# stcodeer/Frequency-wised_All-in-One_Image_Restoration_Model

Measured on AMD Instinct MI355X. Metric: training images/sec @128x128, higher is better.
Workload: dtype bf16; 1 GPU; BASELINE configs[1]: Uformer encoder+decoder (all_3_bands, L=3, freq MSA), denoise sigma=25, 128x128, phase-2 train step (fwd+bwd+Adam, DropPath on); per_gpu_batch=16, global_batch=16, parallelism=dp1, hip_graph=True

## Files before the change

frequency-wised_all-in-one_image_restoration_model_amd/csrc/fw_elem.hip:

```cpp
#include "fw_common.h"
#include <stdlib.h>

namespace {

constexpr int TPB = 256;
FW_DEV long gtid() { return (long)blockIdx.x * TPB + threadIdx.x; }
FW_DEV long gstride() { return (long)gridDim.x * TPB; }
static inline int grid_for(long n, int cap = 8192) { long g = (n + TPB - 1) / TPB; return (int)(g < 1 ? 1 : (g > cap ? cap : g)); }

template <typename T> FW_DEV void ldvec(const T* p, float* f) {
    unpack16<T>(*reinterpret_cast<const uint4*>(p), f);
}
template <typename T> FW_DEV void stvec(T* p, const float* f) { *reinterpret_cast<uint4*>(p) = pack16<T>(f); }
template <typename T> FW_DEV void ldvec4(const T* p, float* f);
template <> FW_SPEC void ldvec4<float>(const float* p, float* f) { unpack16<float>(*reinterpret_cast<const uint4*>(p), f); }
template <> FW_SPEC void ldvec4<bf16raw>(const bf16raw* p, float* f) {
    const uint2 v = *reinterpret_cast<const uint2*>(p);
    f[0] = __uint_as_float(v.x << 16); f[1] = __uint_as_float(v.x & 0xffff0000u);
    f[2] = __uint_as_float(v.y << 16); f[3] = __uint_as_float(v.y & 0xffff0000u);
}
template <typename T> FW_DEV void stvec4(T* p, const float* f);
template <> FW_SPEC void stvec4<float>(float* p, const float* f) { *reinterpret_cast<uint4*>(p) = pack16<float>(f); }
template <> FW_SPEC void stvec4<bf16raw>(bf16raw* p, const float* f) {
    *reinterpret_cast<uint2*>(p) = make_uint2(pack_bf2(f[0], f[1]), pack_bf2(f[2], f[3]));
// ... 654 lines not shown
            if (k < 9) atomicAdd(dw + (long)c * 9 + (8 - k), sum);
            else atomicAdd(dbias + c, sum);
        }
    }
}

template <typename T>
__global__ void im2col4_kernel(const float* __restrict__ x, long ldx, T* __restrict__ col, int B, int H, int W, int C) {
    const int Ho = H / 2, Wo = W / 2, c4n = C >> 2;
    const long total = (long)B * Ho * Wo * 16 * c4n;
    for (long i = gtid(); i < total; i += gstride()) {
        const int c = (int)(i % c4n) * 4; long t = i / c4n;
        const int tap = (int)(t % 16); t /= 16;
        const int ox = (int)(t % Wo); const int oy = (int)((t / Wo) % Ho); const long b = t / ((long)Wo * Ho);
        const int iy = 2 * oy - 1 + (tap >> 2), ix = 2 * ox - 1 + (tap & 3);
        f32x4 v = f32x4{0.f, 0.f, 0.f, 0.f};
        if (iy >= 0 && iy < H && ix >= 0 && ix < W) v = *reinterpret_cast<const f32x4*>(x + ((b * H + iy) * W + ix) * ldx + c);
        T* d = col + (t * 16 + tap) * (long)C + c;
        if (sizeof(T) == 4) *reinterpret_cast<f32x4*>(d) = v;
        else *reinterpret_cast<uint2*>(d) = make_uint2(pack_bf2(v[0], v[1]), pack_bf2(v[2], v[3]));
    }
}
template <typename T>
__global__ void col2im4_kernel(const T* __restrict__ dcol, float* __restrict__ dx, long lddx, const float* __restrict__ dres, long ldr,
                               int B, int H, int W, int C) {
    const int Ho = H / 2, Wo = W / 2, c4n = C >> 2;
    const long total = (long)B * H * W * c4n;
    for (long i = gtid(); i < total; i += gstride()) {
        const int c = (int)(i % c4n) * 4; const long tok = i / c4n;
        const int x = (int)(tok % W); const int y = (int)((tok / W) % H); const long b = tok / ((long)W * H);
        f32x4 acc = f32x4{0.f, 0.f, 0.f, 0.f};
        if (dres) acc = *reinterpret_cast<const f32x4*>(dres + tok * ldr + c);
        for (int ky = (y + 1) & 1; ky < 4; ky += 2) {
            const int oy = (y + 1 - ky) / 2;
            if (y + 1 - ky < 0 || oy >= Ho) continue;
            for (int kx = (x + 1) & 1; kx < 4; kx += 2) {
                const int ox = (x + 1 - kx) / 2;
                if (x + 1 - kx < 0 || ox >= Wo) continue;
                const T* s = dcol + (((b * Ho + oy) * Wo + ox) * 16 + ky * 4 + kx) * (long)C + c;
                for (int e = 0; e < 4; ++e) acc[e] += TT<T>::ld(s + e);
            }
        }
        *reinterpret_cast<f32x4*>(dx + tok * lddx + c) = acc;
    }
}

template <typename T>
__global__ void pixel_shuffle_kernel(const T* __restrict__ g, const float* __restrict__ bias, float* __restrict__ out, long ldo,
                                     int B, int H, int W, int Cout) {
    const int c4n = Cout >> 2;
    const long total = (long)B * H * W * 4 * c4n;
    for (long i = gtid(); i < total; i += gstride()) {
        const int c = (int)(i % c4n) * 4; long t = i / c4n;
        const int q = (int)(t % 4); t /= 4;
        const int x = (int)(t % W); const int y = (int)((t / W) % H); const long b = t / ((long)W * H);
        const T* s = g + t * 4L * Cout + q * Cout + c;
        float* d = out + ((b * 2 * H + 2 * y + (q >> 1)) * 2 * W + 2 * x + (q & 1)) * ldo + c;
        f32x4 v;
        for (int e = 0; e < 4; ++e) v[e] = TT<T>::ld(s + e) + bias[c + e];
        *reinterpret_cast<f32x4*>(d) = v;
    }
}
template <typename T>
__global__ void pixel_unshuffle_kernel(const float* __restrict__ dout, long ldo, T* __restrict__ dg, int B, int H, int W, int Cout) {
    const int c4n = Cout >> 2;
    const long total = (long)B * H * W * 4 * c4n;
// ... 50 lines not shown
    int tx, ty; long n;
    __device__ EcTiles(int B, int H, int W) : tx((W + EC_TX - 1) / EC_TX), ty((H + EC_TY - 1) / EC_TY) { n = (long)B * tx * ty; }
    __device__ void at(long t, long& b, int& y0, int& x0) const { x0 = (int)(t % tx) * EC_TX; y0 = (int)((t / tx) % ty) * EC_TY; b = t / ((long)tx * ty); }
};
FW_DEV void ec_patch_load(float (&r)[EC_PREG], const float* __restrict__ src, const EcTiles& T, long t, int H, int W) {
    long b; int y0, x0;
    T.at(t, b, y0, x0);
#pragma unroll
    for (int k = 0; k < EC_PREG; ++k) {
        int i = threadIdx.x + k * 256; i = i < EC_PN ? i : EC_PN - 1;
        const int ci = i / EC_PLANE, rem = i % EC_PLANE;
        const int y = y0 + rem / EC_PW - 1, x = x0 + rem % EC_PW - 1;
        const bool ok = y >= 0 && y < H && x >= 0 && x < W;
        const int yc = y < 0 ? 0 : (y >= H ? H - 1 : y), xc = x < 0 ? 0 : (x >= W ? W - 1 : x);
        const float v = src[((b * 3 + ci) * H + yc) * W + xc];
        r[k] = ok ? v : 0.f;
    }
}
FW_DEV void ec_patch_store(const float (&r)[EC_PREG], float* patch) {
#pragma unroll
    for (int k = 0; k < EC_PREG; ++k) { const int i = threadIdx.x + k * 256; if (i < EC_PN) patch[i] = r[k]; }
}

template <int MODE>
__global__ __launch_bounds__(256) void edge_conv3_rows_kernel(const float* __restrict__ src, const float* __restrict__ w, const float* __restrict__ bias,
                                                              float* __restrict__ out, long ldo, int B, int H, int W, int C, float slope) {
    __shared__ float patch[2][EC_PN];
    const int c4n = C >> 2, PL = 256 / c4n;
    const int q = threadIdx.x % c4n, pl = threadIdx.x / c4n;
    f32x4 wr[27], bq = f32x4{0.f, 0.f, 0.f, 0.f};
#pragma unroll
    for (int t = 0; t < 27; ++t)
#pragma unroll
        for (int e = 0; e < 4; ++e)
            wr[t][e] = MODE == 0 ? w[(4 * q + e) * 27 + t] : w[((long)(t / 9) * C + 4 * q + e) * 9 + 8 - t % 9];
    if (MODE == 0) bq = *reinterpret_cast<const f32x4*>(bias + 4 * q);
    const EcTiles T(B, H, W);
    float pr[EC_PREG];
    long t = blockIdx.x;
    if (t < T.n) { ec_patch_load(pr, src, T, t, H, W); ec_patch_store(pr, patch[0]); }
    __syncthreads();
    for (int cur = 0; t < T.n; t += gridDim.x, cur ^= 1) {
        const bool more = t + gridDim.x < T.n;
        if (more) ec_patch_load(pr, src, T, t + gridDim.x, H, W);
        long b; int y0, x0;
        T.at(t, b, y0, x0);
        const float* pc = patch[cur];
        if (pl < PL)
            for (int p = pl; p < EC_PIX; p += PL) {
                const int ty = p / EC_TX, tx = p % EC_TX, y = y0 + ty, x = x0 + tx;
                const float* pp = pc + ty * EC_PW + tx;
                f32x4 acc = bq;
#pragma unroll
                for (int ky = 0; ky < 3; ++ky)
#pragma unroll
                    for (int kx = 0; kx < 3; ++kx)
#pragma unroll
                        for (int ci = 0; ci < 3; ++ci) {
                            const int py = MODE == 0 ? ky : 2 - ky, px = MODE == 0 ? kx : 2 - kx;
                            acc += wr[ci * 9 + py * 3 + px] * pp[ci * EC_PLANE + py * EC_PW + px];
                        }
                if (MODE == 0)
#pragma unroll
                    for (int e = 0; e < 4; ++e) acc[e] = lrelu_f(acc[e], slope);
                if (y < H && x < W) *reinterpret_cast<f32x4*>(out + ((b * H + y) * W + x) * ldo + 4 * q) = acc;
            }
        if (more) ec_patch_store(pr, patch[cur ^ 1]);
        __syncthreads();
    }
}

template <int V, int MODE>
__global__ __launch_bounds__(256, 2) void edge_conv3_wgrad_kernel(const float* __restrict__ src, const float* __restrict__ a, long lda, const float* __restrict__ o,
                                                                  long ldo, float* __restrict__ dw, float* __restrict__ db, int B, int H, int W, int C, float slope) {
    constexpr int U = 4;
    __shared__ float patch[2][EC_PN];
    __shared__ float red[28 * 256];
    const int cvn = C / V, PL = 256 / cvn;
    const int q = threadIdx.x % cvn, pl = threadIdx.x / cvn;
    float g[27][V], gb[V];
#pragma unroll
    for (int e = 0; e < V; ++e) {
        gb[e] = 0.f;
#pragma unroll
        for (int t = 0; t < 27; ++t) g[t][e] = 0.f;
    }
    const EcTiles T(B, H, W);
    float pr[EC_PREG];
// ... 429 lines not shown
            ? dwconv_tile_launch<bf16raw, 1>((const bf16raw*)dh2, ldg, w, (const float*)nullptr, (const bf16raw*)h1, (bf16raw*)dh1, (bf16raw*)nullptr, ldo, B, H, W, C, ST)
            : dwconv_tile_launch<float, 1>((const float*)dh2, ldg, w, (const float*)nullptr, (const float*)h1, (float*)dh1, (float*)nullptr, ldo, B, H, W, C, ST);
        if (rc) return rc;
    }
    if (dtype == FW_DT_BF16) {
        if (!tiled) hipLaunchKernelGGL((dwconv_strip_kernel<bf16raw, 1>), dim3((grid_for(n) + 7) / 8 * 8), dim3(TPB), 0, ST, (const bf16raw*)dh2, ldg, w, (const float*)nullptr,
                           (const bf16raw*)h1, (bf16raw*)dh1, (bf16raw*)nullptr, ldo, B, H, W, C);
        if (g1) hipLaunchKernelGGL((dwconv_wgrad_kernel<bf16raw, false>), gridw, dim3(256), 0, ST, (const bf16raw*)dh2, ldg, (const bf16raw*)g1, ld1, dw, dbias, B, H, W, C, NSTRIP);
        else hipLaunchKernelGGL((dwconv_wgrad_kernel<bf16raw, true>), gridw, dim3(256), 0, ST, (const bf16raw*)dh2, ldg, (const bf16raw*)h1, ld1, dw, dbias, B, H, W, C, NSTRIP);
    } else {
        if (!tiled) hipLaunchKernelGGL((dwconv_strip_kernel<float, 1>), dim3((grid_for(n) + 7) / 8 * 8), dim3(TPB), 0, ST, (const float*)dh2, ldg, w, (const float*)nullptr,
                           (const float*)h1, (float*)dh1, (float*)nullptr, ldo, B, H, W, C);
        if (g1) hipLaunchKernelGGL((dwconv_wgrad_kernel<float, false>), gridw, dim3(256), 0, ST, (const float*)dh2, ldg, (const float*)g1, ld1, dw, dbias, B, H, W, C, NSTRIP);
        else hipLaunchKernelGGL((dwconv_wgrad_kernel<float, true>), gridw, dim3(256), 0, ST, (const float*)dh2, ldg, (const float*)h1, ld1, dw, dbias, B, H, W, C, NSTRIP);
    }
    FW_LAUNCH_RET();
}
extern "C" int fw_im2col4(int dtype, const float* x, long ldx, void* col, int B, int H, int W, int C, void* stream) {
    FW_CHECK_ARG(x && col && C % 4 == 0 && ldx % 4 == 0 && H % 2 == 0 && W % 2 == 0);
    const long n = (long)B * (H / 2) * (W / 2) * 16 * (C / 4);
    if (dtype == FW_DT_BF16) LAUNCH((im2col4_kernel<bf16raw>), n, x, ldx, (bf16raw*)col, B, H, W, C);
    LAUNCH((im2col4_kernel<float>), n, x, ldx, (float*)col, B, H, W, C);
}
extern "C" int fw_col2im4(int dtype, const void* dcol, float* dx, long lddx, const float* dres, long ldr, int B, int H, int W, int C,
                          void* stream) {
    FW_CHECK_ARG(dcol && dx && C % 4 == 0 && lddx % 4 == 0 && H % 2 == 0 && W % 2 == 0 && (!dres || ldr % 4 == 0));
    const long n = (long)B * H * W * (C / 4);
    if (dtype == FW_DT_BF16) LAUNCH((col2im4_kernel<bf16raw>), n, (const bf16raw*)dcol, dx, lddx, dres, ldr, B, H, W, C);
    LAUNCH((col2im4_kernel<float>), n, (const float*)dcol, dx, lddx, dres, ldr, B, H, W, C);
}
extern "C" int fw_pixel_shuffle(int dtype, const void* g, const float* bias, float* out, long ldo, int B, int H, int W, int Cout,
                                void* stream) {
    FW_CHECK_ARG(g && bias && out && Cout % 4 == 0 && ldo % 4 == 0);
    const long n = (long)B * H * W * Cout;
    if (dtype == FW_DT_BF16) LAUNCH((pixel_shuffle_kernel<bf16raw>), n, (const bf16raw*)g, bias, out, ldo, B, H, W, Cout);
    LAUNCH((pixel_shuffle_kernel<float>), n, (const float*)g, bias, out, ldo, B, H, W, Cout);
}
extern "C" int fw_pixel_unshuffle(int dtype, const float* dout, long ldo, void* dg, int B, int H, int W, int Cout, void* stream) {
    FW_CHECK_ARG(dout && dg && Cout % 4 == 0 && ldo % 4 == 0);
    const long n = (long)B * H * W * Cout;
    if (dtype == FW_DT_BF16) LAUNCH((pixel_unshuffle_kernel<bf16raw>), n, dout, ldo, (bf16raw*)dg, B, H, W, Cout);
    LAUNCH((pixel_unshuffle_kernel<float>), n, dout, ldo, (float*)dg, B, H, W, Cout);
}
extern "C" int fw_colsum(int x_dtype, const void* x, long ldx, float* out, long rows, int cols, void* stream) {
    FW_CHECK_ARG(x && out && rows > 0 && cols > 0);
    int rpb = (int)((rows + 1023) / 1024);
    if (rpb < 32) rpb = 32;
    int grid = (int)((rows + rpb - 1) / rpb);
    if (x_dtype != 1 && cols % 4 == 0 && cols <= 512 && ldx % 4 == 0 && ((uintptr_t)x & 15) == 0 && ((uintptr_t)out & 3) == 0) {
        rpb = (int)((rows + 255) / 256);
        if (rpb < 32) rpb = 32;
        grid = (int)((rows + rpb - 1) / rpb);
        hipLaunchKernelGGL(colsum4_kernel, dim3(grid), dim3(TPB), 0, ST, (const float*)x, ldx, out, rows, cols, rpb);
        FW_LAUNCH_RET();
    }
    if (x_dtype == 1) hipLaunchKernelGGL((colsum_t_kernel<bf16raw>), dim3(grid), dim3(TPB), 0, ST, (const bf16raw*)x, ldx, out, rows, cols, rpb);
    else hipLaunchKernelGGL(colsum_kernel, dim3(grid), dim3(TPB), 0, ST, (const float*)x, ldx, out, rows, cols, rpb);
    FW_LAUNCH_RET();
}
#ifndef FW_EC_WGRAD_CAP
#define FW_EC_WGRAD_CAP 512
#endif
static inline int ec_grid(int B, int H, int W, int cap) {
    const long n = (long)B * ((H + EC_TY - 1) / EC_TY) * ((W + EC_TX - 1) / EC_TX);
    return (int)(n < cap ? n : cap);
}
static inline bool ec_al16(const void* p) { return ((uintptr_t)p & 15) == 0; }
constexpr int OP_PROD_BYTES = ((EC_PLANE + 15) / 16) * 16 * OP_PS * 4;
constexpr int OP_MAX_C = 896;
extern "C" int fw_inproj_fwd(const float* img, const float* w, const float* bias, float* out, long ldo, int B, int H, int W, int C,
                             float slope, void* stream) {
    FW_CHECK_ARG(img && w && bias && out && C % 4 == 0 && ldo % 4 == 0 && C > 0 && C <= 1024 && B > 0 && H > 0 && W > 0);
    FW_CHECK_ARG(ec_al16(out) && ec_al16(bias));
    hipLaunchKernelGGL(edge_conv3_rows_kernel<0>, dim3(ec_grid(B, H, W, 768)), dim3(TPB), 0, ST, img, w, bias, out, ldo, B, H, W, C, slope);
    FW_LAUNCH_RET();
}
extern "C" int fw_inproj_bwd(const float* img, const float* out, long ldo, const float* dy, long ldy, float* dw, float* db, int B,
                             int H, int W, int C, float slope, void* stream) {
    FW_CHECK_ARG(img && out && dy && dw && db && C > 0 && B > 0 && H > 0 && W > 0);
    const dim3 grid(ec_grid(B, H, W, FW_EC_WGRAD_CAP));
    const bool v4 = C % 4 == 0 && ldo % 4 == 0 && ldy % 4 == 0 && ec_al16(out) && ec_al16(dy);
    const int slice = v4 ? 1024 : 256;
    for (int c0 = 0; c0 < C; c0 += slice) {
        const int cs = C - c0 < slice ? C - c0 : slice;
        if (v4) hipLaunchKernelGGL((edge_conv3_wgrad_kernel<4, 0>), grid, dim3(TPB), 0, ST, img, dy + c0, ldy, out + c0, ldo, dw + (long)c0 * 27, db + c0, B, H, W, cs, slope);
        else hipLaunchKernelGGL((edge_conv3_wgrad_kernel<1, 0>), grid, dim3(TPB), 0, ST, img, dy + c0, ldy, out + c0, ldo, dw + (long)c0 * 27, db + c0, B, H, W, cs, slope);
    }
    FW_LAUNCH_RET();
}
extern "C" int fw_outproj_fwd(const float* fea, long ldf, const float* w, const float* bias, const float* img, float* out, int B,
                              int H, int W, int C, void* stream) {
    FW_CHECK_ARG(fea && w && bias && out && C % 4 == 0 && ldf % 4 == 0 && C > 0 && C <= OP_MAX_C && B > 0 && H > 0 && W > 0 && ec_al16(fea));
    const size_t lds = (size_t)((C + 15) / 16) * 2048 + OP_PROD_BYTES;
    FW_SET_LDS_ONCE(outproj_fwd_mfma_kernel, (OP_MAX_C / 16) * 2048 + OP_PROD_BYTES);
    hipLaunchKernelGGL(outproj_fwd_mfma_kernel, dim3(ec_grid(B, H, W, 512)), dim3(TPB), lds, ST, fea, ldf, w, bias, img, out, B, H, W, C);
    FW_LAUNCH_RET();
}
extern "C" int fw_outproj_bwd(const float* dout, const float* fea, long ldf, const float* w, float* dfea, long lddf, float* dw,
                              float* db, int B, int H, int W, int C, void* stream) {
    FW_CHECK_ARG(dout && fea && w && dfea && dw && db && C % 4 == 0 && ldf % 4 == 0 && lddf % 4 == 0 && C > 0 && C <= 1024 && B > 0 && H > 0 && W > 0);
    FW_CHECK_ARG(ec_al16(fea) && ec_al16(dfea));
    hipLaunchKernelGGL(edge_conv3_rows_kernel<1>, dim3(ec_grid(B, H, W, 768)), dim3(TPB), 0, ST, dout, w, (const float*)nullptr, dfea, lddf, B, H, W, C, 0.f);
    hipLaunchKernelGGL((edge_conv3_wgrad_kernel<4, 1>), dim3(ec_grid(B, H, W, FW_EC_WGRAD_CAP)), dim3(TPB), 0, ST, dout, fea, ldf, (const float*)nullptr, 0L, dw, db,
                       B, H, W, C, 0.f);
    FW_LAUNCH_RET();
}
extern "C" int fw_l1_loss(const float* a, const float* b, float* da, long n, float gscale, float* loss, void* stream) {
    FW_CHECK_ARG(a && b && loss && n > 0);
    hipLaunchKernelGGL(l1_loss_kernel, dim3(grid_for(n, 1024)), dim3(TPB), 0, ST, a, b, da, n, gscale, loss);
    FW_LAUNCH_RET();
}
extern "C" int fw_ce0_loss(const float* logits, float* dlogits, int R, int N, float gscale, float* loss, void* stream) {
    FW_CHECK_ARG(logits && loss && R > 0 && N > 0);
    hipLaunchKernelGGL(ce0_loss_kernel, dim3(R), dim3(64), 0, ST, logits, dlogits, R, N, gscale, loss);
    FW_LAUNCH_RET();
}
extern "C" int fw_adam_tick(float* hyper, float b1, float b2, void* stream) {
    FW_CHECK_ARG(hyper);
    hipLaunchKernelGGL(adam_tick_kernel, dim3(1), dim3(1), 0, ST, hyper, b1, b2);
    FW_LAUNCH_RET();
}
extern "C" int fw_adam(int shadow_dtype, float* p, const float* g, float* m, float* v, void* shadow, long n, const float* hyper,
                       float b1, float b2, float eps, void* stream) {
    FW_CHECK_ARG(p && g && m && v && hyper && n > 0);
    if (shadow_dtype == FW_DT_BF16 && shadow) LAUNCH((adam_kernel<bf16raw>), n, p, g, m, v, (bf16raw*)shadow, n, hyper, b1, b2, eps);
    LAUNCH((adam_kernel<float>), n, p, g, m, v, (float*)shadow, n, hyper, b1, b2, eps);
}
extern "C" int fw_ema(int shadow_dtype, float* pk, const float* pq, void* shadow, long n, float momentum, void* stream) {
// ... 46 lines not shown
```

frequency-wised_all-in-one_image_restoration_model_amd/fwair/functional.py:

```python
import weakref

import torch

from . import ops
from .lib import call, dt


class config:
    compute_dtype = torch.float32
    shadow_epoch = 0
    direct_grads = False


def act_empty(rows, cols, dtype, device):
    ld = (cols + 7) // 8 * 8
    return torch.empty((rows, ld), dtype=dtype, device=device)[:, :cols]


def aligned(t):
    if t.stride(1) == 1 and (t.stride(0) * t.element_size()) % 16 == 0 and t.data_ptr() % 16 == 0:
        return t
    out = act_empty(t.shape[0], t.shape[1], t.dtype, t.device)
    out.copy_(t)
    return out
# ... 432 lines not shown
        else:
            ctx.save_for_backward(h1, weight, wt)
        ctx.bias = bias
        ctx.geo = (B, H, W)
        ctx.mark_non_differentiable(g2)
        return h2, g2

    @staticmethod
    def backward(ctx, dh2, _):
        if dh2 is None:
            return (None,) * 8
        h1, weight, wt = ctx.saved_tensors[:3]
        g1 = ctx.saved_tensors[3] if len(ctx.saved_tensors) > 3 else None
        B, H, W = ctx.geo
        C = h1.shape[1]
        dh2 = aligned(dh2)
        db, rb = _grad_target(ctx.bias)
        dw, rw = _grad_target(weight, (C, 9))
        dh1 = act_empty(h1.shape[0], C, h1.dtype, h1.device)
        call('fw_dwconv_bwd', dt(h1.dtype), dh2, dh2.stride(0), g1, h1, h1.stride(0), wt, dh1, dh1.stride(0), dw, db, B, H, W, C)
        return dh1, None, (rw.view_as(weight) if rw is not None else None), rb, None, None, None, None


class DownsampleFn(torch.autograd.Function):

    @staticmethod
    def forward(ctx, x, weight, bias, B, H, W):
        C, Co = x.shape[1], weight.shape[0]
        col = ops.im2col4(x, B, H, W, config.compute_dtype)
        y = torch.empty((col.shape[0], Co), dtype=torch.float32, device=x.device)
        ops.gemm(col, shadow(weight, 'conv4'), col.shape[0], Co, 16 * C, out=y, bias=bias)
        ctx.save_for_backward(x, weight)
        ctx.bias = bias
        ctx.geo = (B, H, W)
        return y

    @staticmethod
    def backward(ctx, dy):
        x, weight = ctx.saved_tensors
        B, H, W = ctx.geo
        C, Co = x.shape[1], weight.shape[0]
        Mo = dy.shape[0]
        g = ops.cast_rows(dy, config.compute_dtype) if config.compute_dtype != torch.float32 else aligned(dy)
        col = ops.im2col4(x, B, H, W, config.compute_dtype)
        dwk = _zeros((Co, 16 * C), x.device)
        db, rb = _grad_target(ctx.bias)
        ops.wgrad(g, col, Co, 16 * C, Mo, dwk, db)
        dw, rw = _grad_target(weight, (Co, C, 16))
        ops.permute3(dwk, dw, (Co, 16, C), (16 * C, 1, 16), accumulate=True)
        del col
        dcol = ops.gemm(g, shadow(weight, 'conv4'), Mo, 16 * C, Co, w_trans=True)
        dx = ops.col2im4(dcol, B, H, W, C)
        return dx, (rw.view_as(weight) if rw is not None else None), rb, None, None, None


class UpsampleCatFn(torch.autograd.Function):

    @staticmethod
    def forward(ctx, x, skip, weight, bias, B, H, W):
        Cin, Cout = weight.shape[0], weight.shape[1]
        Cs = skip.shape[1]
        xq = ops.cast_rows(x, config.compute_dtype) if config.compute_dtype != torch.float32 else x
        g = ops.gemm(xq, shadow(weight, 'convT2'), x.shape[0], 4 * Cout, Cin)
        out = torch.empty((4 * x.shape[0], Cout + Cs), dtype=torch.float32, device=x.device)
        ops.pixel_shuffle(g, bias, out[:, :Cout], B, H, W, Cout)
        ops.copy_rows(skip, out[:, Cout:])
        ctx.save_for_backward(x, weight)
        ctx.bias = bias
        ctx.geo = (B, H, W, Cs)
        return out

    @staticmethod
    def backward(ctx, dcat):
        x, weight = ctx.saved_tensors
        B, H, W, Cs = ctx.geo
        Cin, Cout = weight.shape[0], weight.shape[1]
        M = x.shape[0]
        dg = ops.pixel_unshuffle(dcat[:, :Cout], B, H, W, Cout, config.compute_dtype)
        xq = ops.cast_rows(x, config.compute_dtype) if config.compute_dtype != torch.float32 else x
        dwt = _zeros((4 * Cout, Cin), x.device)
        ops.wgrad(dg, xq, 4 * Cout, Cin, M, dwt)
        dw, rw = _grad_target(weight, (Cin, Cout, 4))
        ops.permute3(dwt, dw, (4, Cout, Cin), (1, 4, Cout * 4), accumulate=True)
        dx = ops.gemm(dg, shadow(weight, 'convT2'), M, Cin, 4 * Cout, w_trans=True, out_dtype=torch.float32)
        db, rb = _grad_target(ctx.bias)
        ops.colsum(dcat[:, :Cout], db)
        dskip = torch.empty((dcat.shape[0], Cs), dtype=torch.float32, device=x.device)
        ops.copy_rows(dcat[:, Cout:], dskip)
        return dx, dskip, (rw.view_as(weight) if rw is not None else None), rb, None, None, None


class InputProjFn(torch.autograd.Function):
    @staticmethod
    def forward(ctx, img, weight, bias):
        B, _, H, W = img.shape
        C = weight.shape[0]
        img = img.contiguous()
        out = torch.empty((B * H * W, C), dtype=torch.float32, device=img.device)
        call('fw_inproj_fwd', img, weight, bias, out, C, B, H, W, C, 0.01)
        ctx.save_for_backward(img, weight, out)
        return out

    @staticmethod
    def backward(ctx, dy):
        img, weight, out = ctx.saved_tensors
        B, _, H, W = img.shape
        C = weight.shape[0]
        dw, db = _zeros(weight.shape, img.device), _zeros((C,), img.device)
        dy = dy.contiguous()
        call('fw_inproj_bwd', img, out, C, dy, dy.stride(0), dw, db, B, H, W, C, 0.01)
        return None, dw, db


class OutputProjFn(torch.autograd.Function):
    @staticmethod
    def forward(ctx, fea, weight, bias, img):
        B, _, H, W = img.shape
        C = fea.shape[1]
        img = img.contiguous()
        out = torch.empty_like(img)
        call('fw_outproj_fwd', fea, fea.stride(0), weight, bias, img, out, B, H, W, C)
        ctx.save_for_backward(fea, weight)
        ctx.geo = (B, H, W)
        return out

    @staticmethod
    def backward(ctx, dout):
        fea, weight = ctx.saved_tensors
        B, H, W = ctx.geo
        C = fea.shape[1]
        dout = dout.contiguous()
        dfea = torch.empty((fea.shape[0], C), dtype=torch.float32, device=fea.device)
        dw, db = _zeros(weight.shape, fea.device), _zeros((3,), fea.device)
        call('fw_outproj_bwd', dout, fea, fea.stride(0), weight, dfea, C, dw, db, B, H, W, C)
        return dfea, dw, db, None


class BnLreluGapFn(torch.autograd.Function):

    @staticmethod
    def forward(ctx, fea, gamma, beta, rmean, rvar, nbt, B, training):
        ED = gamma.shape[0]
        P = fea.numel() // (B * ED)
        assert fea.is_contiguous()
        dev = fea.device
        gap = torch.empty((B, ED), dtype=torch.float32, device=dev)
        part = torch.empty((ED, B, 2), dtype=torch.float32, device=dev) if training else None
        saved = torch.empty((ED, 2), dtype=torch.float32, device=dev) if training else None
        call('fw_bn_lrelu_gap_fwd', dt(fea.dtype), fea, gamma, beta, rmean, rvar, nbt, part, saved, gap, B, ED, P, int(training),
             1e-5, 0.1, 0.1)
        ctx.save_for_backward(fea, gamma, beta, saved)
        ctx.geo = (B, ED, P, training)
        return gap

    @staticmethod
    def backward(ctx, dgap):
        fea, gamma, beta, saved = ctx.saved_tensors
# ... 325 lines not shown
```

frequency-wised_all-in-one_image_restoration_model_amd/fwair/modules.py:

```python
import math

import os

import torch
import torch.nn as nn

from . import functional as Fn
from . import ops
from .lib import call

WIN = 8
_LEFF_FUSED_MIN_ROWS = int(os.environ.get('FW_LEFF_FUSED_MIN_ROWS', str(1 << 62)))


def trunc_normal_(t, std=.02):
    return nn.init.trunc_normal_(t, std=std)


def _tokens_hw(rows, batch):
    hw = rows // batch
    h = int(math.isqrt(hw))
    assert h * h == hw
    return h

# ... 39 lines not shown
        B, HW, C = x.shape
        xn = Fn.CastFn.apply(x.reshape(B * HW, C))
        h1 = Fn.linear(xn, self.linear1[0].weight, self.linear1[0].bias)
        h2, g2 = Fn.DwConvFn.apply(h1, None, self.conv[0].weight, self.conv[0].bias, B, int(math.isqrt(HW)), int(math.isqrt(HW)))
        y = Fn.linear(g2, self.linear2[0].weight, self.linear2[0].bias, x_pre=h2, out_f32=True)
        return y.view(B, HW, C)


def _rel_index():
    ch = torch.arange(WIN)
    coords = torch.stack(torch.meshgrid([ch, ch], indexing='ij')).flatten(1)
    rel = (coords[:, :, None] - coords[:, None, :]).permute(1, 2, 0).contiguous()
    rel[:, :, 0] += WIN - 1
    rel[:, :, 1] += WIN - 1
    rel[:, :, 0] *= 2 * WIN - 1
    return rel.sum(-1)


class Downsample(nn.Module):
    def __init__(self, in_channel, out_channel):
        super().__init__()
        self.conv = nn.Sequential(nn.Conv2d(in_channel, out_channel, kernel_size=4, stride=2, padding=1))

    def run(self, x, batch):
        h = _tokens_hw(x.shape[0], batch)
        return Fn.DownsampleFn.apply(x, self.conv[0].weight, self.conv[0].bias, batch, h, h)


class Upsample(nn.Module):
    def __init__(self, in_channel, out_channel):
        super().__init__()
        self.deconv = nn.Sequential(nn.ConvTranspose2d(in_channel, out_channel, kernel_size=2, stride=2))

    def run_cat(self, x, skip, batch):
        h = _tokens_hw(x.shape[0], batch)
        return Fn.UpsampleCatFn.apply(x, skip, self.deconv[0].weight, self.deconv[0].bias, batch, h, h)


class InputProj(nn.Module):
    def __init__(self, in_channel=3, out_channel=64):
        super().__init__()
        self.proj = nn.Sequential(nn.Conv2d(in_channel, out_channel, kernel_size=3, stride=1, padding=1), nn.LeakyReLU(inplace=True))

    def run(self, img):
        return Fn.InputProjFn.apply(img, self.proj[0].weight, self.proj[0].bias)


class OutputProj(nn.Module):
    def __init__(self, in_channel=64, out_channel=3):
# ... 210 lines not shown
    def forward(self, x, inter, mask=None):
        assert mask is None
        B = x.shape[0]
        if x.shape[-1] != self.reso or x.shape[-2] != self.reso:
            raise NotImplementedError(f'the decoder is built for {self.reso}x{self.reso} inputs (decoder_Uformer.py:836)')
        coefs = iter(self._coefs(inter, B))
        x = x.contiguous().float()
        y = self.input_proj.run(x)

        visual_freqs = [] if self.debug_mode else None

        def layer(name, t):
            vis = None
            if visual_freqs is not None:
                vis = []
                visual_freqs.append(vis)
            for blk in getattr(self, name).blocks:
                t = blk.run(t, B, next(coefs), vis)
            return t

        conv = []
        for i in range(4):
            y = layer(f'encoderlayer_{i}', y)
            conv.append(y)
            y = getattr(self, f'dowsample_{i}').run(y, B)
        y = layer('bottleneck_0', y)
        y = layer('bottleneck_1', y)
        for i in reversed(range(4)):
            y = getattr(self, f'upsample_{i}').run_cat(y, conv[i], B)
            y = layer(f'decoderlayer_{i}', y)
        out = self.output_proj.run(y, x)
        if self.debug_mode:
            return out, visual_freqs
        return out


class EncWindowAttention(nn.Module):

    def __init__(self, dim, win_size, num_heads):
        super().__init__()
        self.dim, self.win_size, self.num_heads = dim, win_size, num_heads
        self.relative_position_bias_table = nn.Parameter(torch.zeros((2 * win_size[0] - 1) * (2 * win_size[1] - 1), num_heads))
        self.register_buffer('relative_position_index', _rel_index())
        trunc_normal_(self.relative_position_bias_table)
        self.qkv = LinearProjection(dim, num_heads, dim // num_heads)
        self.proj = nn.Linear(dim, dim)

    def tables(self):
# ... 259 lines not shown
```

frequency-wised_all-in-one_image_restoration_model_amd/fwair/ops.py:

```python
import bisect

import torch

from . import lfs as _lfs
from .lib import call, dt, lib


def _ld(t):
    assert t.dim() == 2 and t.stride(1) == 1, 'expect a row-major 2-D view'
    return t.stride(0)


def empty(rows, cols, dtype, device):
    return torch.empty((rows, cols), dtype=dtype, device=device)


def gemm(x, w, M, N, K, *, x_trans=False, w_trans=False, x_op=0, w_op=0, out=None, out_dtype=None, bias=None,
         act=0, slope=0.0, aux=None, rowscale=None, rows_per_scale=1, residual=None, accumulate=False, splitk=1,
         alpha=1.0, out_gelu=None, xsum=None, c_zstride=0, xsum_zstride=0):
    assert x.dtype == w.dtype
    if out is None:
        out = torch.empty((M, N), dtype=out_dtype or x.dtype, device=x.device)
    if accumulate:
        _note_write(out)
# ... 393 lines not shown


def dwconv_fwd(src, w, bias, B, H, W, in_gelu=False):
    h2, g2 = torch.empty_like(src), torch.empty_like(src)
    call('fw_dwconv_fwd', dt(src.dtype), src, _ld(src), int(in_gelu), w, bias, h2, g2, _ld(h2), B, H, W, src.shape[1])
    return h2, g2


def dwconv_bwd(dh2, g1, h1, w, dw, dbias, B, H, W):
    dh1 = torch.empty_like(h1)
    _note_write(dw)
    _note_write(dbias)
    call('fw_dwconv_bwd', dt(h1.dtype), dh2, _ld(dh2), g1, h1, _ld(h1), w, dh1, _ld(dh1), dw, dbias, B, H, W, h1.shape[1])
    return dh1


def im2col4(x, B, H, W, dtype):
    C = x.shape[1]
    col = torch.empty((B * (H // 2) * (W // 2), 16 * C), dtype=dtype, device=x.device)
    call('fw_im2col4', dt(dtype), x, _ld(x), col, B, H, W, C)
    return col


def col2im4(dcol, B, H, W, C, dres=None):
    dx = torch.empty((B * H * W, C), dtype=torch.float32, device=dcol.device)
    call('fw_col2im4', dt(dcol.dtype), dcol, dx, _ld(dx), dres, _ld(dres) if dres is not None else 0, B, H, W, C)
    return dx


def pixel_shuffle(g, bias, out, B, H, W, Cout):
    call('fw_pixel_shuffle', dt(g.dtype), g, bias, out, _ld(out), B, H, W, Cout)
    return out


def pixel_unshuffle(dout, B, H, W, Cout, dtype):
    dg = torch.empty((B * H * W, 4 * Cout), dtype=dtype, device=dout.device)
    call('fw_pixel_unshuffle', dt(dtype), dout, _ld(dout), dg, B, H, W, Cout)
    return dg


def colsum(x, out):
    _note_write(out)
    call('fw_colsum', 1 if x.dtype == torch.bfloat16 else 0, x, _ld(x), out, x.shape[0], x.shape[1])


def cast_rows(src, dtype, rowscale=None, rows_per_scale=1):
    dst = torch.empty(src.shape, dtype=dtype, device=src.device)
    call('fw_cast_rows', dt(dtype), src, _ld(src), dst, _ld(dst), src.shape[0], src.shape[1], rowscale, rows_per_scale)
    return dst
# ... 16 lines not shown
```

include/fwair.h:

```cpp
#ifndef FWAIR_H
#define FWAIR_H
#ifdef __cplusplus
extern "C" {
#endif

int fw_gemm(int dtype, const void* X, long ldx, int x_trans, int x_op, const void* W, long ldw, int w_trans, int w_op,
            void* C, long ldc, int out_f32, int accumulate, int M, int N, int K, float alpha, const float* bias, int act,
            float slope, const void* aux, long ldaux, const float* rowscale, int rows_per_scale, const float* residual,
            long ldr, int splitk, void* C2, long ldc2, float* xsum, long c_zstride, long xsum_zstride, void* stream);
int fw_gemm_last_kernel(char* buf, int n);

int fw_wgrad_group_prob_bytes(void);
int fw_wgrad_group(const void* tab, void* probs, int nprob, const void* items, int nitems, int tile, void* stream);

int fw_slab_reduce(const float* slab, int nz, long n, long zstride, float* dst, int accumulate, float* dst2, long off2, long n2,
                   void* stream);
int fw_slab_reduce_multi(const void* tab, const void* prefix, int num, long total_blocks, void* stream);

int fw_layernorm_fwd(int dtype, const float* x, long ldx, const float* gamma, const float* beta, void* y, long ldy,
                     float* mean, float* rstd, int rows, int C, float eps, void* stream);
int fw_layernorm_bwd_blocks(int rows, int C);
int fw_layernorm_bwd(int dtype, const void* dy, long lddy, const float* x, long ldx, const float* gamma, const float* mean,
                     const float* rstd, const float* dres, long lddres, float* dx, long lddx, float* dgamma, float* dbeta,
                     float* partial, int rows, int C, void* stream);
int fw_layernorm_bwd2(int dtype, const void* dy, long lddy, const float* x, long ldx, const float* gamma, const float* mean,
                      const float* rstd, const float* dres, long lddres, float* dx, long lddx, float* dgamma, float* dbeta,
                      float* partial, int rows, int C, void* twin, long ldtw, const float* twscale, int tw_rows_per_scale,
                      void* stream);

int fw_attn_lfs_table_elems(void);
int fw_attn_fwd(int dtype, int D, int nkt, int lfs, const void* q, const void* k, const void* v, long ld, void* out, long ldo,
                float* lse, const float* bias, const float* coef, const void* lfs_tab, int B, int H, int W, int heads, int L,
                int mode, int shift, float scale, void* stream);
int fw_attn_bwd(int dtype, int D, int nkt, int lfs, const void* q, const void* k, const void* v, long ld, const void* out,
                long ldo, const void* dout, long lddo, const float* lse, const float* bias, const float* coef,
                const void* lfs_tab, void* dq, void* dk, void* dv, void* dk2, void* dv2, long ldd, float* dbias,
                float* dcoef, int B, int H, int W, int heads, int L, int mode, int shift, float scale, int dq_pad, void* stream);

int fw_dwconv_fwd(int dtype, const void* in, long ld1, int in_gelu, const float* w, const float* bias, void* h2, void* g2, long ld2, int B,
                  int H, int W, int C, void* stream);
int fw_dwconv_bwd(int dtype, const void* dh2, long ldg, const void* g1, const void* h1, long ld1, const float* w, void* dh1,
                  long ldo, float* dw, float* dbias, int B, int H, int W, int C, void* stream);

int fw_im2col4(int dtype, const float* x, long ldx, void* col, int B, int H, int W, int C, void* stream);
int fw_col2im4(int dtype, const void* dcol, float* dx, long lddx, const float* dres, long ldr, int B, int H, int W, int C,
               void* stream);
int fw_pixel_shuffle(int dtype, const void* g, const float* bias, float* out, long ldo, int B, int H, int W, int Cout,
                     void* stream);
int fw_pixel_unshuffle(int dtype, const float* dout, long ldo, void* dg, int B, int H, int W, int Cout, void* stream);
int fw_colsum(int x_dtype, const void* x, long ldx, float* out, long rows, int cols, void* stream);

int fw_inproj_fwd(const float* img, const float* w, const float* bias, float* out, long ldo, int B, int H, int W, int C,
                  float slope, void* stream);
int fw_inproj_bwd(const float* img, const float* out, long ldo, const float* dy, long ldy, float* dw, float* db, int B, int H,
                  int W, int C, float slope, void* stream);
int fw_outproj_fwd(const float* fea, long ldf, const float* w, const float* bias, const float* img, float* out, int B, int H,
                   int W, int C, void* stream);
int fw_outproj_bwd(const float* dout, const float* fea, long ldf, const float* w, float* dfea, long lddf, float* dw, float* db,
                   int B, int H, int W, int C, void* stream);

int fw_cast_rows(int dtype, const float* src, long lds_, void* dst, long ldd, long rows, int cols, const float* rowscale,
                 int rows_per_scale, void* stream);
int fw_copy_rows(const float* src, long lds_, float* dst, long ldd, long rows, int cols, int accumulate, void* stream);
int fw_add_rows(int dtype, const void* src, long lds_, void* dst, long ldd, long rows, int cols, void* stream);
int fw_cast_flat(int dtype, const float* src, void* dst, long n, void* stream);
int fw_permute3(int in_dtype, int out_dtype, const void* in, void* out, int d0, int d1, int d2, long s0, long s1, long s2,
                int accumulate, void* stream);
int fw_permute3_multi(const void* tab, const void* prefix, int num, long total_blocks, void* stream);
int fw_fill(float* p, long n, float v, void* stream);
int fw_lrelu_fwd(int dtype, const float* x, void* y, long n, float slope, void* stream);
int fw_lrelu_bwd(int dtype, const void* dy, const float* x, float* dx, long n, float slope, void* stream);

int fw_l1_loss(const float* a, const float* b, float* da, long n, float gscale, float* loss, void* stream);
int fw_ce0_loss(const float* logits, float* dlogits, int R, int N, float gscale, float* loss, void* stream);

int fw_adam_tick(float* hyper, float b1, float b2, void* stream);
int fw_adam(int shadow_dtype, float* p, const float* g, float* m, float* v, void* shadow, long n, const float* hyper, float b1,
            float b2, float eps, void* stream);
int fw_ema(int shadow_dtype, float* pk, const float* pq, void* shadow, long n, float momentum, void* stream);

int fw_dft2_fwd(const float* img, float* fr, float* fi, int nimg, int N, void* stream);
int fw_dft2_bands(const float* fr, const float* fi, const float* mask_unshifted, float* out, int nimg, int N, int nbands,
// ... 101 lines not shown
```

Before: 332.8 images/sec.

## Emit bf16 gradient twins from col2im/outproj backward and fuse skip-gradient add

```diff
diff --git a/frequency-wised_all-in-one_image_restoration_model_amd/csrc/fw_elem.hip b/frequency-wised_all-in-one_image_restoration_model_amd/csrc/fw_elem.hip
--- a/frequency-wised_all-in-one_image_restoration_model_amd/csrc/fw_elem.hip
+++ b/frequency-wised_all-in-one_image_restoration_model_amd/csrc/fw_elem.hip
@@ -700,15 +700,19 @@
     }
 }
 template <typename T>
+FW_DEV void twin_store4(T* d, const f32x4 v, float s) {
+    if (sizeof(T) == 4) *reinterpret_cast<f32x4*>(d) = v * s;
+    else *reinterpret_cast<uint2*>(d) = make_uint2(pack_bf2(v[0] * s, v[1] * s), pack_bf2(v[2] * s, v[3] * s));
+}
+template <typename T>
 __global__ void col2im4_kernel(const T* __restrict__ dcol, float* __restrict__ dx, long lddx, const float* __restrict__ dres, long ldr,
-                               int B, int H, int W, int C) {
+                               int B, int H, int W, int C, T* __restrict__ twin, long ldtw, const float* __restrict__ twscale, int twrps) {
     const int Ho = H / 2, Wo = W / 2, c4n = C >> 2;
     const long total = (long)B * H * W * c4n;
     for (long i = gtid(); i < total; i += gstride()) {
         const int c = (int)(i % c4n) * 4; const long tok = i / c4n;
         const int x = (int)(tok % W); const int y = (int)((tok / W) % H); const long b = tok / ((long)W * H);
         f32x4 acc = f32x4{0.f, 0.f, 0.f, 0.f};
-        if (dres) acc = *reinterpret_cast<const f32x4*>(dres + tok * ldr + c);
         for (int ky = (y + 1) & 1; ky < 4; ky += 2) {
             const int oy = (y + 1 - ky) / 2;
             if (y + 1 - ky < 0 || oy >= Ho) continue;
@@ -719,7 +723,9 @@
                 for (int e = 0; e < 4; ++e) acc[e] += TT<T>::ld(s + e);
             }
         }
+        if (dres) acc += *reinterpret_cast<const f32x4*>(dres + tok * ldr + c);
         *reinterpret_cast<f32x4*>(dx + tok * lddx + c) = acc;
+        if (twin) twin_store4<T>(twin + tok * ldtw + c, acc, twscale ? twscale[tok / twrps] : 1.f);
     }
 }
 
@@ -816,9 +822,11 @@
     for (int k = 0; k < EC_PREG; ++k) { const int i = threadIdx.x + k * 256; if (i < EC_PN) patch[i] = r[k]; }
 }
 
-template <int MODE>
+template <int MODE, typename TW = float>
 __global__ __launch_bounds__(256) void edge_conv3_rows_kernel(const float* __restrict__ src, const float* __restrict__ w, const float* __restrict__ bias,
-                                                              float* __restrict__ out, long ldo, int B, int H, int W, int C, float slope) {
+                                                              float* __restrict__ out, long ldo, int B, int H, int W, int C, float slope,
+                                                              TW* __restrict__ twin, long ldtw, const float* __restrict__ twscale,
+                                                              int twrps) {
     __shared__ float patch[2][EC_PN];
     const int c4n = C >> 2, PL = 256 / c4n;
     const int q = threadIdx.x % c4n, pl = threadIdx.x / c4n;
@@ -857,7 +865,11 @@
                 if (MODE == 0)
 #pragma unroll
                     for (int e = 0; e < 4; ++e) acc[e] = lrelu_f(acc[e], slope);
-                if (y < H && x < W) *reinterpret_cast<f32x4*>(out + ((b * H + y) * W + x) * ldo + 4 * q) = acc;
+                if (y < H && x < W) {
+                    const long tok = (b * H + y) * W + x;
+                    *reinterpret_cast<f32x4*>(out + tok * ldo + 4 * q) = acc;
+                    if (MODE == 1 && twin) twin_store4<TW>(twin + tok * ldtw + 4 * q, acc, twscale ? twscale[tok / twrps] : 1.f);
+                }
             }
         if (more) ec_patch_store(pr, patch[cur ^ 1]);
         __syncthreads();
@@ -1333,12 +1345,18 @@
     if (dtype == FW_DT_BF16) LAUNCH((im2col4_kernel<bf16raw>), n, x, ldx, (bf16raw*)col, B, H, W, C);
     LAUNCH((im2col4_kernel<float>), n, x, ldx, (float*)col, B, H, W, C);
 }
+extern "C" int fw_col2im4_tw(int dtype, const void* dcol, float* dx, long lddx, const float* dres, long ldr, int B, int H, int W, int C,
+                             void* twin, long ldtw, const float* twscale, int tw_rows_per_scale, void* stream) {
+    FW_CHECK_ARG(dcol && dx && C % 4 == 0 && lddx % 4 == 0 && H % 2 == 0 && W % 2 == 0 && (!dres || ldr % 4 == 0));
+    FW_CHECK_ARG(!twin || (ldtw % 4 == 0 && (!twscale || tw_rows_per_scale > 0)));
+    const long n = (long)B * H * W * (C / 4);
+    if (dtype == FW_DT_BF16)
+        LAUNCH((col2im4_kernel<bf16raw>), n, (const bf16raw*)dcol, dx, lddx, dres, ldr, B, H, W, C, (bf16raw*)twin, ldtw, twscale, tw_rows_per_scale);
+    LAUNCH((col2im4_kernel<float>), n, (const float*)dcol, dx, lddx, dres, ldr, B, H, W, C, (float*)twin, ldtw, twscale, tw_rows_per_scale);
+}
 extern "C" int fw_col2im4(int dtype, const void* dcol, float* dx, long lddx, const float* dres, long ldr, int B, int H, int W, int C,
                           void* stream) {
-    FW_CHECK_ARG(dcol && dx && C % 4 == 0 && lddx % 4 == 0 && H % 2 == 0 && W % 2 == 0 && (!dres || ldr % 4 == 0));
-    const long n = (long)B * H * W * (C / 4);
-    if (dtype == FW_DT_BF16) LAUNCH((col2im4_kernel<bf16raw>), n, (const bf16raw*)dcol, dx, lddx, dres, ldr, B, H, W, C);
-    LAUNCH((col2im4_kernel<float>), n, (const float*)dcol, dx, lddx, dres, ldr, B, H, W, C);
+    return fw_col2im4_tw(dtype, dcol, dx, lddx, dres, ldr, B, H, W, C, nullptr, 0, nullptr, 1, stream);
 }
 extern "C" int fw_pixel_shuffle(int dtype, const void* g, const float* bias, float* out, long ldo, int B, int H, int W, int Cout,
                                 void* stream) {
@@ -1383,7 +1401,8 @@
                              float slope, void* stream) {
     FW_CHECK_ARG(img && w && bias && out && C % 4 == 0 && ldo % 4 == 0 && C > 0 && C <= 1024 && B > 0 && H > 0 && W > 0);
     FW_CHECK_ARG(ec_al16(out) && ec_al16(bias));
-    hipLaunchKernelGGL(edge_conv3_rows_kernel<0>, dim3(ec_grid(B, H, W, 768)), dim3(TPB), 0, ST, img, w, bias, out, ldo, B, H, W, C, slope);
+    hipLaunchKernelGGL((edge_conv3_rows_kernel<0, float>), dim3(ec_grid(B, H, W, 768)), dim3(TPB), 0, ST, img, w, bias, out, ldo, B, H, W, C, slope,
+                       (float*)nullptr, 0L, (const float*)nullptr, 1);
     FW_LAUNCH_RET();
 }
 extern "C" int fw_inproj_bwd(const float* img, const float* out, long ldo, const float* dy, long ldy, float* dw, float* db, int B,
@@ -1407,14 +1426,25 @@
     hipLaunchKernelGGL(outproj_fwd_mfma_kernel, dim3(ec_grid(B, H, W, 512)), dim3(TPB), lds, ST, fea, ldf, w, bias, img, out, B, H, W, C);
     FW_LAUNCH_RET();
 }
-extern "C" int fw_outproj_bwd(const float* dout, const float* fea, long ldf, const float* w, float* dfea, long lddf, float* dw,
-                              float* db, int B, int H, int W, int C, void* stream) {
+extern "C" int fw_outproj_bwd_tw(const float* dout, const float* fea, long ldf, const float* w, float* dfea, long lddf, float* dw,
+                                 float* db, int B, int H, int W, int C, int tw_dtype, void* twin, long ldtw, const float* twscale,
+                                 int tw_rows_per_scale, void* stream) {
     FW_CHECK_ARG(dout && fea && w && dfea && dw && db && C % 4 == 0 && ldf % 4 == 0 && lddf % 4 == 0 && C > 0 && C <= 1024 && B > 0 && H > 0 && W > 0);
     FW_CHECK_ARG(ec_al16(fea) && ec_al16(dfea));
-    hipLaunchKernelGGL(edge_conv3_rows_kernel<1>, dim3(ec_grid(B, H, W, 768)), dim3(TPB), 0, ST, dout, w, (const float*)nullptr, dfea, lddf, B, H, W, C, 0.f);
+    FW_CHECK_ARG(!twin || (ldtw % 4 == 0 && (!twscale || tw_rows_per_scale > 0) && ((uintptr_t)twin & 7) == 0));
+    if (twin && tw_dtype == FW_DT_BF16)
+        hipLaunchKernelGGL((edge_conv3_rows_kernel<1, bf16raw>), dim3(ec_grid(B, H, W, 768)), dim3(TPB), 0, ST, dout, w, (const float*)nullptr, dfea, lddf,
+                           B, H, W, C, 0.f, (bf16raw*)twin, ldtw, twscale, tw_rows_per_scale);
+    else
+        hipLaunchKernelGGL((edge_conv3_rows_kernel<1, float>), dim3(ec_grid(B, H, W, 768)), dim3(TPB), 0, ST, dout, w, (const float*)nullptr, dfea, lddf,
+                           B, H, W, C, 0.f, (float*)twin, ldtw, twscale, tw_rows_per_scale);
     hipLaunchKernelGGL((edge_conv3_wgrad_kernel<4, 1>), dim3(ec_grid(B, H, W, FW_EC_WGRAD_CAP)), dim3(TPB), 0, ST, dout, fea, ldf, (const float*)nullptr, 0L, dw, db,
                        B, H, W, C, 0.f);
     FW_LAUNCH_RET();
+}
+extern "C" int fw_outproj_bwd(const float* dout, const float* fea, long ldf, const float* w, float* dfea, long lddf, float* dw,
+                              float* db, int B, int H, int W, int C, void* stream) {
+    return fw_outproj_bwd_tw(dout, fea, ldf, w, dfea, lddf, dw, db, B, H, W, C, FW_DT_F32, nullptr, 0, nullptr, 1, stream);
 }
 extern "C" int fw_l1_loss(const float* a, const float* b, float* da, long n, float gscale, float* loss, void* stream) {
     FW_CHECK_ARG(a && b && loss && n > 0);
diff --git a/frequency-wised_all-in-one_image_restoration_model_amd/fwair/functional.py b/frequency-wised_all-in-one_image_restoration_model_amd/fwair/functional.py
--- a/frequency-wised_all-in-one_image_restoration_model_amd/fwair/functional.py
+++ b/frequency-wised_all-in-one_image_restoration_model_amd/fwair/functional.py
@@ -478,10 +478,19 @@
         return dh1, None, (rw.view_as(weight) if rw is not None else None), rb, None, None, None, None
 
 
+def _twin_of(dy, dtype, shape):
+    tw = getattr(dy, '_fw_twin', None)
+    if tw is not None and tw[1] is None and tw[0].dtype == dtype and tw[0].shape == shape:
+        return tw[0]
+    return None
+
+
 class DownsampleFn(torch.autograd.Function):
 
     @staticmethod
-    def forward(ctx, x, weight, bias, B, H, W):
+    def forward(ctx, x, weight, bias, B, H, W, want_skip=False):
+        ctx.set_materialize_grads(False)
+        ctx.rs_hint = getattr(x, '_fw_rs', None)
         C, Co = x.shape[1], weight.shape[0]
         col = ops.im2col4(x, B, H, W, config.compute_dtype)
         y = torch.empty((col.shape[0], Co), dtype=torch.float32, device=x.device)
@@ -489,15 +498,24 @@
         ctx.save_for_backward(x, weight)
         ctx.bias = bias
         ctx.geo = (B, H, W)
+        if want_skip:
+            return y, x.view_as(x)
         return y
 
     @staticmethod
-    def backward(ctx, dy):
+    def backward(ctx, dy, dskip=None):
+        if dy is None:
+            return dskip, None, None, None, None, None, None
         x, weight = ctx.saved_tensors
         B, H, W = ctx.geo
         C, Co = x.shape[1], weight.shape[0]
         Mo = dy.shape[0]
-        g = ops.cast_rows(dy, config.compute_dtype) if config.compute_dtype != torch.float32 else aligned(dy)
+        if config.compute_dtype != torch.float32:
+            g = _twin_of(dy, config.compute_dtype, (Mo, Co))
+            if g is None:
+                g = ops.cast_rows(dy, config.compute_dtype)
+        else:
+            g = aligned(dy)
         col = ops.im2col4(x, B, H, W, config.compute_dtype)
         dwk = _zeros((Co, 16 * C), x.device)
         db, rb = _grad_target(ctx.bias)
@@ -506,8 +524,25 @@
         ops.permute3(dwk, dw, (Co, 16, C), (16 * C, 1, 16), accumulate=True)
         del col
         dcol = ops.gemm(g, shadow(weight, 'conv4'), Mo, 16 * C, Co, w_trans=True)
-        dx = ops.col2im4(dcol, B, H, W, C)
-        return dx, (rw.view_as(weight) if rw is not None else None), rb, None, None, None
+        twin = None
+        if ctx.rs_hint is not None and dcol.dtype != torch.float32:
+            twin = act_empty(x.shape[0], C, dcol.dtype, x.device)
+        rs, rps = ctx.rs_hint if ctx.rs_hint is not None else (None, 1)
+        if dskip is not None and not (dskip.dtype == torch.float32 and dskip.stride(1) == 1 and dskip.stride(0) % 4 == 0
+                                      and dskip.data_ptr() % 16 == 0):
+            dskip = dskip.float().contiguous()
+        dx = ops.col2im4(dcol, B, H, W, C, dres=dskip, twin=twin, twscale=rs, tw_rows_per_scale=rps)
+        if twin is not None:
+            dx._fw_twin = (twin, rs, rps)
+        return dx, (rw.view_as(weight) if rw is not None else None), rb, None, None, None, None
+
+
+def downsample(x, weight, bias, B, H, W, want_skip=False):
+    out = DownsampleFn.apply(x, weight, bias, B, H, W, want_skip)
+    y = out[0] if want_skip else out
+    if y.requires_grad and config.compute_dtype != torch.float32:
+        y._fw_rs = (None, 1)
+    return out
 
 
 class UpsampleCatFn(torch.autograd.Function):
@@ -521,28 +556,26 @@
         out = torch.empty((4 * x.shape[0], Cout + Cs), dtype=torch.float32, device=x.device)
         ops.pixel_shuffle(g, bias, out[:, :Cout], B, H, W, Cout)
         ops.copy_rows(skip, out[:, Cout:])
-        ctx.save_for_backward(x, weight)
+        ctx.save_for_backward(xq, weight)
         ctx.bias = bias
         ctx.geo = (B, H, W, Cs)
         return out
 
     @staticmethod
     def backward(ctx, dcat):
-        x, weight = ctx.saved_tensors
+        xq, weight = ctx.saved_tensors
         B, H, W, Cs = ctx.geo
         Cin, Cout = weight.shape[0], weight.shape[1]
-        M = x.shape[0]
+        M = xq.shape[0]
         dg = ops.pixel_unshuffle(dcat[:, :Cout], B, H, W, Cout, config.compute_dtype)
-        xq = ops.cast_rows(x, config.compute_dtype) if config.compute_dtype != torch.float32 else x
-        dwt = _zeros((4 * Cout, Cin), x.device)
+        dwt = _zeros((4 * Cout, Cin), xq.device)
         ops.wgrad(dg, xq, 4 * Cout, Cin, M, dwt)
         dw, rw = _grad_target(weight, (Cin, Cout, 4))
         ops.permute3(dwt, dw, (4, Cout, Cin), (1, 4, Cout * 4), accumulate=True)
         dx = ops.gemm(dg, shadow(weight, 'convT2'), M, Cin, 4 * Cout, w_trans=True, out_dtype=torch.float32)
         db, rb = _grad_target(ctx.bias)
         ops.colsum(dcat[:, :Cout], db)
-        dskip = torch.empty((dcat.shape[0], Cs), dtype=torch.float32, device=x.device)
-        ops.copy_rows(dcat[:, Cout:], dskip)
+        dskip = dcat[:, Cout:]
         return dx, dskip, (rw.view_as(weight) if rw is not None else None), rb, None, None, None
 
 
@@ -578,6 +611,7 @@
         call('fw_outproj_fwd', fea, fea.stride(0), weight, bias, img, out, B, H, W, C)
         ctx.save_for_backward(fea, weight)
         ctx.geo = (B, H, W)
+        ctx.rs_hint = getattr(fea, '_fw_rs', None)
         return out
 
     @staticmethod
@@ -588,7 +622,14 @@
         dout = dout.contiguous()
         dfea = torch.empty((fea.shape[0], C), dtype=torch.float32, device=fea.device)
         dw, db = _zeros(weight.shape, fea.device), _zeros((3,), fea.device)
-        call('fw_outproj_bwd', dout, fea, fea.stride(0), weight, dfea, C, dw, db, B, H, W, C)
+        twin = None
+        if ctx.rs_hint is not None and config.compute_dtype != torch.float32:
+            twin = act_empty(fea.shape[0], C, config.compute_dtype, fea.device)
+        rs, rps = ctx.rs_hint if ctx.rs_hint is not None else (None, 1)
+        call('fw_outproj_bwd_tw', dout, fea, fea.stride(0), weight, dfea, C, dw, db, B, H, W, C,
+             dt(twin.dtype) if twin is not None else 0, twin, twin.stride(0) if twin is not None else 0, rs, rps)
+        if twin is not None:
+            dfea._fw_twin = (twin, rs, rps)
         return dfea, dw, db, None
 
 
diff --git a/frequency-wised_all-in-one_image_restoration_model_amd/fwair/modules.py b/frequency-wised_all-in-one_image_restoration_model_amd/fwair/modules.py
--- a/frequency-wised_all-in-one_image_restoration_model_amd/fwair/modules.py
+++ b/frequency-wised_all-in-one_image_restoration_model_amd/fwair/modules.py
@@ -85,9 +85,9 @@
         super().__init__()
         self.conv = nn.Sequential(nn.Conv2d(in_channel, out_channel, kernel_size=4, stride=2, padding=1))
 
-    def run(self, x, batch):
+    def run(self, x, batch, want_skip=False):
         h = _tokens_hw(x.shape[0], batch)
-        return Fn.DownsampleFn.apply(x, self.conv[0].weight, self.conv[0].bias, batch, h, h)
+        return Fn.downsample(x, self.conv[0].weight, self.conv[0].bias, batch, h, h, want_skip)
 
 
 class Upsample(nn.Module):
@@ -344,8 +344,8 @@
         conv = []
         for i in range(4):
             y = layer(f'encoderlayer_{i}', y)
-            conv.append(y)
-            y = getattr(self, f'dowsample_{i}').run(y, B)
+            y, skip = getattr(self, f'dowsample_{i}').run(y, B, want_skip=True)
+            conv.append(skip)
         y = layer('bottleneck_0', y)
         y = layer('bottleneck_1', y)
         for i in reversed(range(4)):
diff --git a/frequency-wised_all-in-one_image_restoration_model_amd/fwair/ops.py b/frequency-wised_all-in-one_image_restoration_model_amd/fwair/ops.py
--- a/frequency-wised_all-in-one_image_restoration_model_amd/fwair/ops.py
+++ b/frequency-wised_all-in-one_image_restoration_model_amd/fwair/ops.py
@@ -439,9 +439,11 @@
     return col
 
 
-def col2im4(dcol, B, H, W, C, dres=None):
+def col2im4(dcol, B, H, W, C, dres=None, twin=None, twscale=None, tw_rows_per_scale=1):
     dx = torch.empty((B * H * W, C), dtype=torch.float32, device=dcol.device)
-    call('fw_col2im4', dt(dcol.dtype), dcol, dx, _ld(dx), dres, _ld(dres) if dres is not None else 0, B, H, W, C)
+    assert twin is None or twin.dtype == dcol.dtype
+    call('fw_col2im4_tw', dt(dcol.dtype), dcol, dx, _ld(dx), dres, _ld(dres) if dres is not None else 0, B, H, W, C,
+         twin, _ld(twin) if twin is not None else 0, twscale, tw_rows_per_scale)
     return dx
 
 
diff --git a/include/fwair.h b/include/fwair.h
--- a/include/fwair.h
+++ b/include/fwair.h
@@ -45,6 +45,8 @@
 int fw_im2col4(int dtype, const float* x, long ldx, void* col, int B, int H, int W, int C, void* stream);
 int fw_col2im4(int dtype, const void* dcol, float* dx, long lddx, const float* dres, long ldr, int B, int H, int W, int C,
                void* stream);
+int fw_col2im4_tw(int dtype, const void* dcol, float* dx, long lddx, const float* dres, long ldr, int B, int H, int W, int C,
+                  void* twin, long ldtw, const float* twscale, int tw_rows_per_scale, void* stream);
 int fw_pixel_shuffle(int dtype, const void* g, const float* bias, float* out, long ldo, int B, int H, int W, int Cout,
                      void* stream);
 int fw_pixel_unshuffle(int dtype, const float* dout, long ldo, void* dg, int B, int H, int W, int Cout, void* stream);
@@ -58,6 +60,9 @@
                    int W, int C, void* stream);
 int fw_outproj_bwd(const float* dout, const float* fea, long ldf, const float* w, float* dfea, long lddf, float* dw, float* db,
                    int B, int H, int W, int C, void* stream);
+int fw_outproj_bwd_tw(const float* dout, const float* fea, long ldf, const float* w, float* dfea, long lddf, float* dw, float* db,
+                      int B, int H, int W, int C, int tw_dtype, void* twin, long ldtw, const float* twscale, int tw_rows_per_scale,
+                      void* stream);
 
 int fw_cast_rows(int dtype, const float* src, long lds_, void* dst, long ldd, long rows, int cols, const float* rowscale,
                  int rows_per_scale, void* stream);
```

Result: no change. 334.7 images/sec (median of 6 runs) (+0.6%).
